# gvtulder/elasticdeform

Hardware: AMD Instinct MI355X
Metric: Mvoxels/s fwd+grad, 256^3 fp32 order=3 (higher is better)
Workload: dtype f32; 1 GPU; cfg2: 3D 256x256x256 float32, 5x5x5 grid sigma 5, order 3, mode mirror, prefilter on, deform_grid + deform_grid_gradient per step, one volume per GPU; parallelism=1 volume per GPU, no collective

## Files before the change

### elasticdeform_amd/csrc/deform_k1z.hip

```cpp
#include <hip/hip_runtime.h>

#include <cstring>
#include <type_traits>

#include "ed_device.h"
#include "ed_gridfilter.h"
#include "ed_params.h"
#include "ed_tile.h"
#include "ed_workspace.h"
#include "ed_zwalk.h"

namespace ed {
namespace tile {

#ifdef EDHIP_K1_STATS
__device__ unsigned long long g_k1z_stats[8];
#define ZSTAT(K, N) atomicAdd(&g_k1z_stats[K], (unsigned long long)(N))
#else
#define ZSTAT(K, N) do { } while (0)
#endif

namespace {


enum : int {
    kZAny = 1,
    kZStaged = 2,
    kZFast = 4,
    kZDma = 8,
    kZXin = 16,
    kZZYin = 32,
    kZUnfit = 64,
    kZGen = 128,
};
struct ZRecU {
    int b0z, b0y, b0x, flags, pitch, ez, ey, ex, goff, plane;
};
typedef int zv8i __attribute__((ext_vector_type(8)));
typedef const __attribute__((address_space(4))) zv8i* crec_p;
__device__ __forceinline__ ZRecU zrec_unpack(const zv8i& v)
{
    ZRecU r;
    r.b0z = v[0];
    r.b0y = v[1];
    r.b0x = v[2];
    r.flags = v[3];
    r.pitch = (v[3] >> 8) & 255;
    r.ez = v[4] & 1023;
    r.ey = (v[4] >> 10) & 1023;
    r.ex = (int)((unsigned)v[4] >> 20);
    r.goff = v[5];
    r.plane = r.ey * r.pitch;
    return r;
}
__device__ __forceinline__ ZRecU zrec_load(crec_p p)
{
    const zv8i v = *p;
    return zrec_unpack(v);
}

__host__ __device__ __forceinline__ int zctl(int parity, int list, int xcd) { return (parity * 2 + list) * 8 + xcd; }

#define ED_RED6(CTRL)                                      \
    "v_min_i32_dpp %0, %0, %0 " CTRL "\n\t"                \
    "v_min_i32_dpp %1, %1, %1 " CTRL "\n\t"                \
    "v_min_i32_dpp %2, %2, %2 " CTRL "\n\t"                \
    "v_max_i32_dpp %3, %3, %3 " CTRL "\n\t"                \
    "v_max_i32_dpp %4, %4, %4 " CTRL "\n\t"                \
    "v_max_i32_dpp %5, %5, %5 " CTRL "\n\t"
__device__ __forceinline__ void zrow_box(int (&lo)[3], int (&hi)[3])
{
    asm volatile("s_nop 1\n\t"
                 ED_RED6("quad_perm:[1,0,3,2] row_mask:0xf bank_mask:0xf")
                 ED_RED6("quad_perm:[2,3,0,1] row_mask:0xf bank_mask:0xf")
                 ED_RED6("row_half_mirror row_mask:0xf bank_mask:0xf")
                 ED_RED6("row_mirror row_mask:0xf bank_mask:0xf")
                 : "+v"(lo[0]), "+v"(lo[1]), "+v"(lo[2]), "+v"(hi[0]), "+v"(hi[1]), "+v"(hi[2]));
}
#undef ED_RED6
__device__ __forceinline__ int zuni(int v) { return __builtin_amdgcn_readfirstlane(v); }
__device__ __forceinline__ void zlds_barrier() { asm volatile("s_waitcnt lgkmcnt(0)\n\ts_barrier" ::: "memory"); }
__device__ __forceinline__ void zdma_barrier() { asm volatile("s_waitcnt vmcnt(0) lgkmcnt(0)\n\ts_barrier" ::: "memory"); }
__device__ __forceinline__ void zglds16(const float* g, float* lds)
{
    __builtin_amdgcn_global_load_lds((const __attribute__((address_space(1))) void*)g,
                                     (__attribute__((address_space(3))) void*)lds, 16, 0, 0);
}
template <bool OUT16>
__device__ __forceinline__ void zstore_out(float* img, long long off, float val, int io16)
{
    if constexpr (OUT16)
        reinterpret_cast<unsigned short*>(img)[off] = (unsigned short)narrow16(val, io16);
    else
        __builtin_nontemporal_store(val, img + off);
}

__device__ __forceinline__ void zaxis_entry(const GridGeom& g, int a, int oi, double* w, int* idx)
{
    const double cp = control_coordinate(g.ncp[a], (int64_t)oi + g.off[a], g.in_len[a]);
    const int64_t start = window_start(cp, 3);
    const bool edge = start < 0 || start + 3 >= g.ncp[a];
    spline_weights(cp, 3, w);
#pragma unroll
    for (int l = 0; l < 4; ++l)
        idx[l] = edge ? mirror_i32((int)start + l, (int)g.ncp[a]) : (int)start + l;
}

constexpr int kGeoBlock = 256;
constexpr int kGeoWaves = kGeoBlock / 64;
__global__ __launch_bounds__(kGeoBlock) void k1z_geo_kernel(const GridGeom g, const HotGeom hg, const ZGeom zg,
                                                          const GridPrefilter gp)
{
    extern __shared__ __attribute__((aligned(16))) char smem[];
    const int tid = threadIdx.x;
// ... 190 lines not shown
            lo[h] = (int)floor(cr - slack[h]);
            hi[h] = (int)floor(cr + slack[h]);
        }
        bool out_of_fast = false;
#pragma unroll
        for (int h = 0; h < 3; ++h)
            out_of_fast = out_of_fast || lo[h] < ((order & 1) ? 0 : 1) || hi[h] > hg.in_len[h] - 2;
        const bool fast = nz == kT && ny == kT && nx == kT && !__any(out_of_fast);
        zrow_box(lo, hi);
        int* dst = sBox + (tz * 8 + (lane >> 4)) * 8;
        if ((lane & 15) == 0) {
#pragma unroll
            for (int h = 0; h < 3; ++h) {
                dst[h] = lo[h];
                dst[4 + h] = hi[h];
            }
        }
        if (lane == 0)
            dst[3] = fast ? 1 : 0;
        if (!fast) {
            bool cst = false;
#pragma unroll
            for (int h = 0; h < 3; ++h) {
                double m = c[h];
                if (!(m >= 0.0 && m <= (double)(hg.in_len[h] - 1)))
                    m = map_coordinate_fast(m, hg.in_len[h], hg.mode, hg.period[h], hg.inv_period[h]);
                cst = cst || !(m > -1.0);
                const double mr = (order & 1) ? m : m + 0.5;
                lo[h] = (int)floor(mr - slack[h]);
                hi[h] = (int)floor(mr + slack[h]);
            }
            if (cst) {
#pragma unroll
                for (int h = 0; h < 3; ++h) {
                    lo[h] = 0x7fffffff;
                    hi[h] = (int)0x80000000;
                }
            }
            zrow_box(lo, hi);
            if ((lane & 15) == 0) {
#pragma unroll
                for (int h = 0; h < 3; ++h) {
                    dst[32 + h] = lo[h];
                    dst[36 + h] = hi[h];
                }
            }
        }
    }
    __syncthreads();
    ZTICK(6);
    for (int tz = tid; tz < hg.tiles[0] && !ED_DBG(hg.dbg, 1 << 27); tz += kGeoBlock) {
        const int tile_id = sample * hg.ntiles + (tz * hg.tiles[1] + ty) * hg.tiles[2] + tx;
        int cls = 0;
        bool hint0 = false, half_fit[2] = {false, false};
#pragma unroll 1
        for (int part = 0; part < 3; ++part) {
            const int* sb = sBox + tz * 64;
            const bool fast = sb[3] != 0;
            const int r0 = part == 2 ? 2 : 0, r1 = part == 1 ? 2 : 3;
            int blo[3], bhi[3];
            bool any = true;
#pragma unroll
            for (int h = 0; h < 3; ++h) {
                int rlo = 0x7fffffff, rhi = (int)0x80000000, lo = 0x7fffffff, hi = (int)0x80000000;
                for (int r = r0; r <= r1; ++r) {
                    rlo = min(rlo, sb[r * 8 + h]);
                    rhi = max(rhi, sb[r * 8 + 4 + h]);
                    lo = min(lo, sb[(fast ? 0 : 32) + r * 8 + h]);
                    hi = max(hi, sb[(fast ? 0 : 32) + r * 8 + 4 + h]);
                }
                if (!fast) {
                    any = any && hi >= lo;
                    const int lowfold = hg.mode == EDHIP_MODE_REFLECT ? -1 : 0;
                    if (rlo < ((order & 1) ? 0 : 1) && rhi >= lowfold)
                        lo = min(lo, lowfold);
                    if (rhi > hg.in_len[h] - 2 && rlo <= hg.in_len[h] - 1)
                        hi = max(hi, hg.in_len[h] - 1);
                }
                blo[h] = lo - H;
                bhi[h] = hi - H + order + (h == 2 ? kPadX : 0);
            }
            if (!any) {
                blo[0] = blo[1] = blo[2] = 0;
                bhi[0] = bhi[1] = bhi[2] = -1;
            }
            any = bhi[0] >= blo[0] && bhi[1] >= blo[1] && bhi[2] >= blo[2];
            unsigned ext[3];
#pragma unroll
            for (int h = 0; h < 3; ++h)
                ext[h] = (unsigned)bhi[h] - (unsigned)blo[h] + 1u;
            const int pitch = ext[2] <= 16u ? 16 : (ext[2] <= 24u ? 24 : (ext[2] <= 32u ? 32 : (ext[2] <= 48u ? 48 : 0)));
            const bool sane = any && ext[0] < 1024u && ext[1] < 1024u;
            const int nrows = sane ? (int)(ext[0] * ext[1]) : 0;
            const bool fits = sane && pitch > 0 && nrows * pitch <= hg.box_cap;
            const bool dma = fits && blo[2] >= 0 && blo[2] + pitch + 1 <= hg.in_len[2];
            const bool xin = fits && blo[2] >= 0 && blo[2] + (int)ext[2] <= hg.in_len[2];
            const bool zyin = fits && blo[0] >= 0 && blo[0] + (int)ext[0] <= hg.in_len[0] && blo[1] >= 0 &&
                              blo[1] + (int)ext[1] <= hg.in_len[1];
            const bool fastA = part == 0 && fast && fits && dma && zyin;
            const int flags = (any ? kZAny : 0) | (fits ? kZStaged : 0) | (fastA ? kZFast : kZGen) | (dma ? kZDma : 0) |
                              (xin ? kZXin : 0) | (zyin ? kZZYin : 0) | (any && !fits ? kZUnfit : 0);
            const int4 w0 = make_int4(blo[0], blo[1], blo[2], flags | (pitch << 8));
            const int4 w1 = make_int4(sane ? (int)(ext[0] | (ext[1] << 10) | (ext[2] << 20)) : 0,
                                      (dma && zyin) ? blo[0] * hg.vol_sz + blo[1] * hg.vol_sy + blo[2] : 0, 0, 0);
            if (part == 0) {
                hint0 = any && !(sane && pitch > 0 && nrows * pitch <= hg.small_cap);
                cls = (flags & kZUnfit) ? 3 : ((flags & kZFast) ? 1 : 2);
                int4* dst = reinterpret_cast<int4*>(zg.recs + (size_t)tile_id * 8);
                dst[0] = w0;
                dst[1] = w1;
                if (hg.boxes) {
                    int* bx = hg.boxes + (size_t)tile_id * 8;
#pragma unroll
                    for (int h = 0; h < 3; ++h) {
                        bx[h] = blo[h];
                        bx[3 + h] = bhi[h] - ((h == 2 && any) ? kPadX : 0);
                    }
                }
                if (cls != 3)
                    break;
            } else {
                half_fit[part - 1] = fits || !any;
                int4* dst = reinterpret_cast<int4*>(zg.recs_half + ((size_t)tile_id * 2 + (part - 1)) * 8);
                dst[0] = w0;
                dst[1] = w1;
            }
        }
        const bool split = cls == 3 && half_fit[0] && half_fit[1];
        ZSTAT(cls == 3 ? (split ? 6 : 5) : (cls == 1 ? 3 : 4), 1);
        sCls[tz] = cls | (split ? 4 : 0) | (hint0 ? 8 : 0);
    }
    __syncthreads();
    ZTICK(7);
    {
        const int zstrips = (hg.tiles[0] + zg.strip_tiles - 1) / zg.strip_tiles;
        if (tid < 4)
            sCnt[tid] = 0;
        __syncthreads();
        int slotG = -1, slotF = -1, sidv = 0;
        if (tid < zstrips) {
            int info = 0;
            bool g = false, f = false;
            for (int k = 0; k < zg.strip_tiles && tid * zg.strip_tiles + k < hg.tiles[0]; ++k) {
                const int c = sCls[tid * zg.strip_tiles + k];
                info |= c << (4 * k);
                g = g || (c & 3) == 2 || (c & 7) == 7;
                f = f || (c & 7) == 3;
            }
            const size_t sid = (size_t)sample * zg.nstrips + ((size_t)tid * hg.tiles[1] + ty) * hg.tiles[2] + tx;
            sidv = (int)sid;
            zg.sinfo[sid] = info;
            zg.missed[sid] = f ? 2 : 0;
            if (g)
                slotG = atomicAdd(&sCnt[0], 1);
            if (f)
                slotF = atomicAdd(&sCnt[1], 1);
        }
        __syncthreads();
        const int xcd = (tx + ty + sample) & 7;
        if (tid == 0) {
            sCnt[2] = sCnt[0] ? atomicAdd(&zg.ctl[zctl(zg.parity, 0, xcd)], sCnt[0]) : 0;
            sCnt[3] = sCnt[1] ? atomicAdd(&zg.ctl[zctl(zg.parity, 1, xcd)], sCnt[1]) : 0;
        }
        if (blockIdx.x == 0 && sample == 0 && tid < 16)
            zg.ctl[zctl(1 - zg.parity, tid >> 3, tid & 7)] = 0;
        __syncthreads();
        if (slotG >= 0)
            zg.list_g[(size_t)(sCnt[2] + slotG) * 8 + xcd] = sidv;
        if (slotF >= 0)
            zg.list_f[(size_t)(sCnt[3] + slotF) * 8 + xcd] = sidv;
    }
    ZTICK(8);
#undef ZTICK
}


struct ZVox {
    int addr[2];
    float frac[2][3];
    int flg;
};
struct ZStrip {
    int tz0, ty, tx, ntile, sample, id;
};
__device__ __forceinline__ bool k1z_strip(int total_strips, int nstrips, int tiles_z, int tiles_y, int tiles_x, int strip_tiles, int deal,
                                          ZStrip& sp, int b)
{
    const int x = b & 7, j = b >> 3;
    const int r = j / deal;
    int s = (r * 8 + ((x + r) & 7)) * deal + (j - r * deal);
    if (s >= total_strips)
        return false;
    sp.id = s;
    sp.sample = s / nstrips;
    s -= sp.sample * nstrips;
    sp.tx = s % tiles_x;
    s /= tiles_x;
    sp.ty = s % tiles_y;
    sp.tz0 = (s / tiles_y) * strip_tiles;
    sp.ntile = min(strip_tiles, tiles_z - sp.tz0);
    return true;
}
inline unsigned k1z_grid(int total_strips, int deal)
{
    const int chunks = (total_strips + deal - 1) / deal;
    return (unsigned)(((chunks + 7) / 8) * 8 * deal);
}

template <int ORDER, int PITCH>
__device__ __forceinline__ float k1z_gather(const float* bp, int plane, int pitch_rt, const float* w0, const float* w1, const float* w2)
{
    constexpr int NT = ORDER + 1;
    constexpr int NTX = NT + (NT & 1);
    float a0 = 0.f;
#pragma unroll
    for (int l0 = 0; l0 < NT; ++l0) {
        const float* pp = bp + l0 * plane;
        float a1 = 0.f;
#pragma unroll
        for (int l1 = 0; l1 < NT; ++l1) {
            const float* rp = pp + l1 * (PITCH ? PITCH : pitch_rt);
// ... 1 lines not shown
#pragma unroll
            for (int l2 = 0; l2 < NTX; l2 += 2) {
                const float2 pr = *reinterpret_cast<const float2*>(rp + l2);
                ED_NO_DS_MERGE();
                a2 = fmaf(w2[l2], pr.x, a2);
                a2 = fmaf(w2[l2 + 1], pr.y, a2);
            }
            a1 = fmaf(w1[l1], a2, a1);
        }
        a0 = fmaf(w0[l0], a1, a0);
    }
    return a0;
}
template <int ORDER>
__device__ __forceinline__ float k1z_voxel(const char* smem, int addr, const float (&frac)[3], int pitch, int plane)
{
    constexpr int NT = ORDER + 1;
    constexpr int NTX = NT + (NT & 1);
    float f0 = frac[0], f1 = frac[1], f2 = frac[2];
    asm volatile("" : "+v"(f0), "+v"(f1), "+v"(f2));
    float w0[NT], w1[NT], w2[NTX];
    weights_from_frac<float, ORDER>(f0, w0);
    weights_from_frac<float, ORDER>(f1, w1);
    weights_from_frac<float, ORDER>(f2, w2);
    if (NT & 1)
        w2[NT] = 0.f;
    const float* bp = reinterpret_cast<const float*>(smem + addr);
    return pitch == 16 ? k1z_gather<ORDER, 16>(bp, plane, 16, w0, w1, w2) : k1z_gather<ORDER, 0>(bp, plane, pitch, w0, w1, w2);
}

struct ZFast {
    const float* vol;
    float* img;
    const double* r;
    const AxTab* zt;
    const int* recs;
    const int* recs_half;
    int* missed;
    int* hint;
    const int* sinfo;
    const int* list_g;
    int* list_f;
    int* ctl;
    int parity;
    const long long* steps;
    long long vol_bstride, img_bstride, r_bstride;
    int vol_sy, vol_sz, img_sy, img_sz;
    int box_cap, tiles_y, tiles_x, tiles_z, strip_tiles, nstrips, total_strips, ntiles;
    int rcol_bytes, out_y, out_x;
    int kz0, ky0, kx0;
    int io16, nsteps, deal;
    int dbg;
    double aff[12];
};

template <int ORDER, bool AFFINE, bool OUT16, bool STEPS>
__device__ __forceinline__ void k1z_fast_body(const ZFast& a, const int vblock)
{
    constexpr int NT = ORDER + 1;
    constexpr int kPadX = NT & 1;
    constexpr int NTX = NT + kPadX;
    extern __shared__ __attribute__((aligned(16))) char smem[];
    ZStrip sp;
    if (!k1z_strip(a.total_strips, a.nstrips, a.tiles_z, a.tiles_y, a.tiles_x, a.strip_tiles, a.deal, sp, vblock))
        return;
    const int tid = threadIdx.x;
    const int lane = tid & 63;
    const int wave = zuni(tid >> 6);
    const int io16 = OUT16 ? a.io16 : 0;
    const int ntile = sp.ntile;
    const size_t tile_step = (size_t)a.tiles_y * a.tiles_x;
    crec_p rec0 = (crec_p)(const void*)a.recs + ((size_t)sp.sample * a.ntiles + ((size_t)sp.tz0 * a.tiles_y + sp.ty) * a.tiles_x + sp.tx);
    const int sinfo = ((cint_p)(const void*)a.sinfo)[sp.id];
    if (a.hint && tid == 0) {
        const int nh = __builtin_popcount((unsigned)sinfo & 0x88888888u);
        if (nh)
            atomicAdd(a.hint, nh);
    }
    auto next_fast = [&](int t) {
        for (++t; t < ntile; ++t)
            if (((sinfo >> (4 * t)) & 3) == 1)
                break;
        return t;
    };
    int ti = next_fast(-1);
    if (ti >= ntile)
        return;

    const int box_cap = a.box_cap;
    const int odd_shift = (box_cap - 1) * 4;
    float* box0 = reinterpret_cast<float*>(smem);
    float* box1 = box0 + box_cap;
    const int vol_sz = a.vol_sz, vol_sy = a.vol_sy, img_sz = a.img_sz;

    const int yy = lane >> 3, xx = lane & 7;
    const int oy = sp.ty * kT + yy, ox = sp.tx * kT + xx;
    const int obase = oy * a.img_sy + ox;
    const float* __restrict__ vol = a.vol + sp.sample * a.vol_bstride;
    float* img = a.img + sp.sample * a.img_bstride;
    const char* rcol = reinterpret_cast<const char*>(a.r + sp.sample * a.r_bstride) +
                       ((size_t)min(oy, a.out_y - 1) * a.out_x + min(ox, a.out_x - 1)) * (size_t)a.rcol_bytes;
    const int ky = AFFINE ? a.ky0 : oy + a.ky0;
    const int kx = AFFINE ? a.kx0 : ox + a.kx0;
    const int kz0 = a.kz0;
    double Pyx[3];
#pragma unroll
    for (int h = 0; h < 3; ++h)
// ... 59 lines not shown
            const int rx = ci[2] + dx;
            bad |= (rz | ry | rx) | ((ez - rz) | (ey - ry) | (ex - rx));
            const int off = __mul24(rz, rc.plane) + (__mul24(ry, rc.pitch) + rx);
            vs.addr[i] = __mul24(off & 1, odd_shift) + off * 4;
        }
    };

    cll_p steps = (cll_p)(const void*)a.steps;
    ZVox cur, nxt;
    ZRecU rc = zrec_load(rec0 + (size_t)ti * tile_step), rn = rc;
    {
        const ZEnt ze[2] = {k1z_entry(zt, (sp.tz0 + ti) * kT + wave), k1z_entry(zt, (sp.tz0 + ti) * kT + wave + 4)};
        tile_coords(ti, rc, ze, cur);
    }
    while (ti < ntile) {
        const int tn = next_fast(ti);
        const int tl = tn < ntile ? tn : ti;
        const zv8i rnv = *(rec0 + (size_t)tl * tile_step);
        const ZEnt zn[2] = {k1z_entry(zt, (sp.tz0 + tl) * kT + wave), k1z_entry(zt, (sp.tz0 + tl) * kT + wave + 4)};
        if (!ED_DBG(a.dbg, 1 << 18))
            stage(rc, vol + (STEPS ? steps[0] : 0));
        if (tn < ntile) {
            rn = zrec_unpack(rnv);
            tile_coords(tn, rn, zn, nxt);
        }
        const long long ozoff = (long long)((sp.tz0 + ti) * kT + wave) * img_sz + obase;
        const int nsteps = STEPS ? a.nsteps : 1;
        for (int ss = 0; ss < nsteps; ++ss) {
            if (STEPS && ss > 0)
                stage(rc, vol + steps[2 * ss]);
            zdma_barrier();
#pragma unroll
            for (int i = 0; i < 2; ++i) {
                const float val = ED_DBG(a.dbg, 1 << 17) ? cur.frac[i][0] + cur.frac[i][1] + cur.frac[i][2] + __int_as_float(cur.addr[i])
                                                         : k1z_voxel<ORDER>(smem, cur.addr[i], cur.frac[i], rc.pitch, rc.plane);
                if (!ED_DBG(a.dbg, 1 << 20) || val == 123.456f)
                    zstore_out<OUT16>(img, (STEPS ? steps[2 * ss + 1] : 0) + ozoff + (long long)(4 * i) * img_sz, val, io16);
            }
            zlds_barrier();
        }
        cur = nxt;
        rc = rn;
        ti = tn;
    }
    if (__any(bad < 0) && lane == 0) {
        if (atomicOr(a.missed + sp.id, 1) == 0) {
            const int xcd = vblock & 7;
            a.list_f[(size_t)atomicAdd(a.ctl + zctl(a.parity, 1, xcd), 1) * 8 + xcd] = sp.id;
        }
    }
}

template <int ORDER, bool AFFINE, bool OUT16, bool STEPS>
__device__ __forceinline__ void k1z_gen_body(const ZFast& a, czgen_p zn, const int vblock, const int ngen)
{
    constexpr int NT = ORDER + 1;
    constexpr int kPadX = NT & 1;
    constexpr int NTX = NT + kPadX;
    extern __shared__ __attribute__((aligned(16))) char smem[];
    const int tid = threadIdx.x;
    const int lane = tid & 63;
    const int wave = zuni(tid >> 6);
    const int io16 = OUT16 ? a.io16 : 0;
    const int xcd = vblock & 7, nper = ngen >> 3;
    const int nwork = ((cint_p)(const void*)a.ctl)[zctl(a.parity, 0, xcd)];
    if ((vblock >> 3) >= nwork)
        return;
    const int box_cap = a.box_cap;
    const int odd_shift = (box_cap - 1) * 4;
    float* box0 = reinterpret_cast<float*>(smem);
    float* box1 = box0 + box_cap;
    const int vol_sz = a.vol_sz, vol_sy = a.vol_sy, img_sz = a.img_sz;
    const size_t tile_step = (size_t)a.tiles_y * a.tiles_x;
    cdbl_p zt = (cdbl_p)(const void*)a.zt;
    cll_p steps = (cll_p)(const void*)a.steps;
    const int nsteps = STEPS ? a.nsteps : 1;
    const int yy = lane >> 3, xx = lane & 7;

    for (int work = vblock >> 3; work < nwork; work += nper) {
        ZStrip sp;
        {
            int sid = ((cint_p)(const void*)a.list_g)[(size_t)work * 8 + xcd];
            sp.id = sid;
            sp.sample = sid / a.nstrips;
            sid -= sp.sample * a.nstrips;
            sp.tx = sid % a.tiles_x;
            sid /= a.tiles_x;
            sp.ty = sid % a.tiles_y;
            sp.tz0 = (sid / a.tiles_y) * a.strip_tiles;
            sp.ntile = min(a.strip_tiles, a.tiles_z - sp.tz0);
        }
        const int ntile = sp.ntile;
        crec_p rec0 = (crec_p)(const void*)a.recs + ((size_t)sp.sample * a.ntiles + ((size_t)sp.tz0 * a.tiles_y + sp.ty) * a.tiles_x + sp.tx);
        const int sinfo = ((cint_p)(const void*)a.sinfo)[sp.id];
        crec_p rech0 = (crec_p)(const void*)a.recs_half + ((size_t)sp.sample * a.ntiles + ((size_t)sp.tz0 * a.tiles_y + sp.ty) * a.tiles_x + sp.tx) * 2;
        if (tid == 0)
            ZSTAT(7, 1);
        if (work != (vblock >> 3))
            zlds_barrier();
        const int oy = sp.ty * kT + yy, ox = sp.tx * kT + xx;
        const int obase = oy * a.img_sy + ox;
        const float* __restrict__ vol = a.vol + sp.sample * a.vol_bstride;
        float* img = a.img + sp.sample * a.img_bstride;
        const char* rcol = reinterpret_cast<const char*>(a.r + sp.sample * a.r_bstride) +
                           ((size_t)min(oy, a.out_y - 1) * a.out_x + min(ox, a.out_x - 1)) * (size_t)a.rcol_bytes;
        double Pyx[3];
#pragma unroll
        for (int h = 0; h < 3; ++h)
            Pyx[h] = AFFINE ? fma(zn->aff[h * 4 + 2], (double)ox, fma(zn->aff[h * 4 + 1], (double)oy, zn->aff[h * 4 + 3] + zn->offd[h])) : 0.0;
        ZTaps tp;
        tp.key[0] = tp.key[1] = tp.key[2] = tp.key[3] = -1;
        auto stage = [&](const ZRecU& rc, const float* src) {
            const int flags = rc.flags;
            if (!(flags & kZStaged))
                return;
            const int by = rc.ey, pitch = rc.pitch;
            if (flags & kZDma) {
                const int cpr = pitch >> 2, RW = 64 / cpr;
                const int lr = (lane * (65536 / cpr + 1)) >> 16, q = lane - lr * cpr;
                const float* g0 = src + (rc.b0x + 4 * q);
                for (int zrow = wave; zrow < rc.ez; zrow += 4) {
                    const float* gp = g0 + (long long)mirror_i32(rc.b0z + zrow, zn->in_len[0]) * vol_sz;
                    const int lrow0 = zrow * by;
                    for (int y0 = 0; y0 < by; y0 += RW) {
                        if (lr < RW && y0 + lr < by) {
                            const float* g = gp + (long long)mirror_i32(rc.b0y + y0 + lr, zn->in_len[1]) * vol_sy;
                            zglds16(g, box0 + (lrow0 + y0) * pitch);
                            zglds16(g + 1, box1 + (lrow0 + y0) * pitch);
                        }
                    }
                }
            } else {
                const int nrows = rc.ez * rc.ey;
                const float inv_by = __frcp_rn((float)by);
                const int sub = tid & 7;
                for (int rb = tid >> 3; rb < nrows; rb += 2 * (kBlock / 8)) {
                    for (int x0 = sub; x0 < rc.ex; x0 += 16) {
                        float val[2][2];
#pragma unroll
                        for (int u = 0; u < 2; ++u) {
                            const int r = min(rb + u * (kBlock / 8), nrows - 1);
                            const int zrow = (int)(((float)r + 0.5f) * inv_by), yr = r - zrow * by;
                            const int zs = mirror_i32(rc.b0z + zrow, zn->in_len[0]);
                            const int ys = mirror_i32(rc.b0y + yr, zn->in_len[1]);
                            const float* rowp = src + (zs * vol_sz + ys * vol_sy);
#pragma unroll
                            for (int j = 0; j < 2; ++j) {
                                const int xi = min(x0 + 8 * j, rc.ex - 1);
                                const int xs = mirror_i32(rc.b0x + xi, zn->in_len[2]);
                                val[u][j] = rowp[xs];
                            }
                        }
#pragma unroll
                        for (int u = 0; u < 2; ++u) {
                            const int r = rb + u * (kBlock / 8);
#pragma unroll
                            for (int j = 0; j < 2; ++j) {
                                const int xi = x0 + 8 * j;
                                if (r < nrows && xi < rc.ex) {
                                    box0[r * pitch + xi] = val[u][j];
                                    if (xi > 0)
                                        box1[r * pitch + xi - 1] = val[u][j];
                                }
                            }
                        }
                    }
                }
            }
        };
        int bad = 0;
        auto tile_coords = [&](int t, int mask, const ZRecU& rc, ZVox& vs) {
            const int ez = rc.ez - NT, ey = rc.ey - NT, ex = rc.ex - NTX;
            const bool staged = (rc.flags & kZStaged) != 0;
            vs.flg = 0;
#pragma unroll
            for (int i = 0; i < 2; ++i) {
                if (!(mask & (1 << i)))
                    continue;
                const int oz = (sp.tz0 + t) * kT + wave + 4 * i;
                double zw[4];
                k1z_slice(zt, rcol, min(oz, zn->out_len[0] - 1), tp, zw);
                double d[3];
                k1z_disp(tp, zw, d);
                const int b[3] = {oz + zn->off[0], oy + zn->off[1], ox + zn->off[2]};
                double P[3] = {0.0, 0.0, 0.0};
                if (AFFINE) {
#pragma unroll
                    for (int h = 0; h < 3; ++h)
                        P[h] = fma(zn->aff[h * 4 + 0], (double)oz, Pyx[h]);
                }
                int start[3];
                const bool cst = k1z_coords<ORDER, AFFINE>(zn, d, b, P, start, vs.frac[i]);
                const bool valid = oz < zn->out_len[0] && oy < zn->out_len[1] && ox < zn->out_len[2];
                const int rz = start[0] - rc.b0z, ry = start[1] - rc.b0y, rx = start[2] - rc.b0x;
                if (valid && !cst)
                    bad |= staged ? (rz | ry | rx) | ((ez - rz) | (ey - ry) | (ex - rx)) : -1;
                vs.flg |= (valid && !cst && staged ? 1 << i : 0) | (valid && (cst || staged) ? 4 << i : 0);
                const int off = __mul24(rz, rc.plane) + (__mul24(ry, rc.pitch) + rx);
                vs.addr[i] = __mul24(off & 1, odd_shift) + off * 4;
            }
        };
        {
            auto next_item = [&](int it) {
                int t = it >> 1;
                if (it >= 0 && (it & 1) == 0 && ((sinfo >> (4 * t)) & 7) == 7)
                    return it + 1;
                for (++t; t < ntile; ++t) {
                    const int c = (sinfo >> (4 * t)) & 7;
                    if ((c & 3) == 2 || c == 7)
                        break;
                }
                return 2 * t;
            };
            auto item_rec = [&](int it) {
                const int t = it >> 1;
                const bool split = ((sinfo >> (4 * t)) & 7) == 7;
                return zrec_load(split ? rech0 + ((size_t)t * tile_step * 2 + (it & 1)) : rec0 + (size_t)t * tile_step);
            };
            auto item_mask = [&](int it) { return ((sinfo >> (4 * (it >> 1))) & 7) == 7 ? 1 << (it & 1) : 3; };
            ZVox cur, nxt;
            int it = next_item(-2);
            ZRecU rc = item_rec(it < 2 * ntile ? it : 0), rn = rc;
            if (it < 2 * ntile)
                tile_coords(it >> 1, item_mask(it), rc, cur);
            while (it < 2 * ntile) {
                stage(rc, vol + (STEPS ? steps[0] : 0));
                const int in = next_item(it);
                if (in < 2 * ntile) {
                    rn = item_rec(in);
                    tile_coords(in >> 1, item_mask(in), rn, nxt);
                }
                const bool staged = (rc.flags & kZStaged) != 0;
                const long long ozoff = (long long)((sp.tz0 + (it >> 1)) * kT + wave) * img_sz + obase;
                for (int ss = 0; ss < nsteps; ++ss) {
                    if (STEPS && ss > 0)
                        stage(rc, vol + steps[2 * ss]);
                    if (staged)
                        zdma_barrier();
#pragma unroll
                    for (int i = 0; i < 2; ++i) {
                        if (!(cur.flg & (4 << i)))
                            continue;
                        float val = zn->cval;
                        if (cur.flg & (1 << i))
                            val = k1z_voxel<ORDER>(smem, cur.addr[i], cur.frac[i], rc.pitch, rc.plane);
                        zstore_out<OUT16>(img, (STEPS ? steps[2 * ss + 1] : 0) + ozoff + (long long)(4 * i) * img_sz, val, io16);
                    }
                    if (staged)
                        zlds_barrier();
                }
                cur = nxt;
                rc = rn;
                it = in;
            }
        }
        if (__any(bad < 0) && lane == 0) {
            if (atomicOr(a.missed + sp.id, 1) == 0) {
                const int xcd = vblock & 7;
                a.list_f[(size_t)atomicAdd(a.ctl + zctl(a.parity, 1, xcd), 1) * 8 + xcd] = sp.id;
            }
        }
    }
}

template <int ORDER, bool AFFINE, bool OUT16, bool STEPS>
__global__ __launch_bounds__(kBlock, 4) void k1z_tile_kernel(const ZFast a, czgen_p zn, const int ngen, const int every)
{
    const int row = (int)(blockIdx.x >> 3), xcd = (int)(blockIdx.x & 7);
    const int gen_rows = ngen >> 3;
    const int gens_before = min((row + 1) / every, gen_rows);
    const bool is_gen = gens_before > 0 && (row + 1) % every == 0 && (row + 1) / every <= gen_rows;
    if (is_gen)
        k1z_gen_body<ORDER, AFFINE, OUT16, STEPS>(a, zn, (gens_before - 1) * 8 + xcd, ngen);
    else
        k1z_fast_body<ORDER, AFFINE, OUT16, STEPS>(a, (row - gens_before) * 8 + xcd);
}

template <int ORDER, bool AFFINE, bool OUT16, bool STEPS>
__global__ __launch_bounds__(kBlock) void k1z_fix_kernel(const ZFast a, czgen_p zn)
{
    constexpr int NT = ORDER + 1;
    constexpr int kPadX = NT & 1;
    const int tid = threadIdx.x;
    const int lane = tid & 63;
    const int wave = zuni(tid >> 6);
    const int io16 = OUT16 ? a.io16 : 0;
    const int xcd = (int)(blockIdx.x & 7), nper = (int)(gridDim.x >> 3);
    const int nwork = ((cint_p)(const void*)a.ctl)[zctl(a.parity, 1, xcd)];
    if ((int)(blockIdx.x >> 3) >= nwork)
        return;
    const int vol_sz = a.vol_sz, vol_sy = a.vol_sy, img_sz = a.img_sz;
    const size_t tile_step = (size_t)a.tiles_y * a.tiles_x;
    cdbl_p zt = (cdbl_p)(const void*)a.zt;
    cll_p steps = (cll_p)(const void*)a.steps;
    const int nsteps = STEPS ? a.nsteps : 1;
    const int yy = lane >> 3, xx = lane & 7;

    for (int work = blockIdx.x >> 3; work < nwork; work += nper) {
        ZStrip sp;
        {
            int sid = ((cint_p)(const void*)a.list_f)[(size_t)work * 8 + xcd];
            sp.id = sid;
            sp.sample = sid / a.nstrips;
            sid -= sp.sample * a.nstrips;
            sp.tx = sid % a.tiles_x;
            sid /= a.tiles_x;
            sp.ty = sid % a.tiles_y;
            sp.tz0 = (sid / a.tiles_y) * a.strip_tiles;
            sp.ntile = min(a.strip_tiles, a.tiles_z - sp.tz0);
        }
        const int ntile = sp.ntile;
        crec_p rec0 = (crec_p)(const void*)a.recs + ((size_t)sp.sample * a.ntiles + ((size_t)sp.tz0 * a.tiles_y + sp.ty) * a.tiles_x + sp.tx);
        crec_p rech0 = (crec_p)(const void*)a.recs_half + ((size_t)sp.sample * a.ntiles + ((size_t)sp.tz0 * a.tiles_y + sp.ty) * a.tiles_x + sp.tx) * 2;
        const int sinfo = ((cint_p)(const void*)a.sinfo)[sp.id];
        const bool missed = (((cint_p)(const void*)a.missed)[sp.id] & 1) != 0;
        if (!STEPS && false)
            (void)steps;
        const int oy = sp.ty * kT + yy, ox = sp.tx * kT + xx;
        const int obase = oy * a.img_sy + ox;
        const float* __restrict__ vol = a.vol + sp.sample * a.vol_bstride;
        float* img = a.img + sp.sample * a.img_bstride;
        const char* rcol = reinterpret_cast<const char*>(a.r + sp.sample * a.r_bstride) +
                           ((size_t)min(oy, a.out_y - 1) * a.out_x + min(ox, a.out_x - 1)) * (size_t)a.rcol_bytes;
        double Pyx[3];
#pragma unroll
        for (int h = 0; h < 3; ++h)
            Pyx[h] = AFFINE ? fma(zn->aff[h * 4 + 2], (double)ox, fma(zn->aff[h * 4 + 1], (double)oy, zn->aff[h * 4 + 3] + zn->offd[h])) : 0.0;
        ZTaps tp;
// ... 38 lines not shown
                                  rx = (gen ? st[2] : raw[2]) - rc.b0x;
                        const bool inside = rz >= 0 && rz + NT <= rc.ez && ry >= 0 && ry + NT <= rc.ey && rx >= 0 &&
                                            rx + NT + kPadX <= rc.ex;
                        if (inside)
                            continue;
                    }
                    int tap[3][NT];
                    float w[3][NT];
#pragma unroll
                    for (int h = 0; h < 3; ++h) {
                        weights_from_frac<float, ORDER>(fr[h], w[h]);
                        const int stride = h == 0 ? vol_sz : (h == 1 ? vol_sy : 1);
#pragma unroll
                        for (int l = 0; l < NT; ++l)
                            tap[h][l] = mirror_i32(st[h] + l, zn->in_len[h]) * stride;
                    }
                    const long long ooff = (long long)oz * img_sz + obase;
                    ZSTAT(whole ? 2 : 1, 1);
                    for (int ss = 0; ss < nsteps; ++ss) {
                        float val = zn->cval;
                        if (!cst) {
                            const float* src = vol + (STEPS ? steps[2 * ss] : 0);
                            float a0 = 0.f;
#pragma unroll
                            for (int l0 = 0; l0 < NT; ++l0) {
                                float a1 = 0.f;
#pragma unroll
                                for (int l1 = 0; l1 < NT; ++l1) {
                                    const float* p1 = src + (tap[0][l0] + tap[1][l1]);
                                    float a2 = 0.f;
#pragma unroll
                                    for (int l2 = 0; l2 < NT; ++l2)
                                        a2 = fmaf(w[2][l2], p1[tap[2][l2]], a2);
                                    a1 = fmaf(w[1][l1], a2, a1);
                                }
                                a0 = fmaf(w[0][l0], a1, a0);
                            }
                            val = a0;
                        }
                        zstore_out<OUT16>(img, (STEPS ? steps[2 * ss + 1] : 0) + ooff, val, io16);
                    }
                }
            }
        }
    }
}

template <int ORDER, bool AFFINE, bool OUT16, bool STEPS>
hipError_t launch_k1z_kernels(const ZFast& zf, const void* znp, unsigned ngen, unsigned nfix, size_t lds, hipStream_t stream)
{
    const unsigned nfast = k1z_grid(zf.total_strips, zf.deal);
    const unsigned fast_rows = nfast >> 3, gen_rows = ngen >> 3;
    unsigned every = gen_rows ? fast_rows / gen_rows + 1 : 2;
    if (every < 2)
        every = 2;
    hipLaunchKernelGGL((k1z_tile_kernel<ORDER, AFFINE, OUT16, STEPS>), dim3(nfast + ngen), dim3(kBlock), lds, stream, zf, (czgen_p)znp,
                       (int)ngen, (int)every);
    hipError_t e = hipGetLastError();
    if (e != hipSuccess)
        return e;
    hipLaunchKernelGGL((k1z_fix_kernel<ORDER, AFFINE, OUT16, STEPS>), dim3(nfix, 2 * zf.strip_tiles), dim3(kBlock), 0, stream, zf, (czgen_p)znp);
    return hipGetLastError();
}
template <int ORDER, bool AFFINE, bool OUT16>
hipError_t launch_k1z_variant(const ZFast& zf, const void* zn, unsigned ngen, unsigned nfix, size_t lds, hipStream_t stream,
                              bool steps)
{
    return steps ? launch_k1z_kernels<ORDER, AFFINE, OUT16, true>(zf, zn, ngen, nfix, lds, stream)
                 : launch_k1z_kernels<ORDER, AFFINE, OUT16, false>(zf, zn, ngen, nfix, lds, stream);
}
template <int ORDER>
hipError_t launch_k1z_order(const HotGeom& hg, const ZFast& zf, const void* zn, unsigned ngen, unsigned nfix, size_t lds, hipStream_t stream)
{
    const bool steps = hg.nstep != 0;
    if (hg.io16)
        return hg.has_affine ? launch_k1z_variant<ORDER, true, true>(zf, zn, ngen, nfix, lds, stream, steps)
                             : launch_k1z_variant<ORDER, false, true>(zf, zn, ngen, nfix, lds, stream, steps);
    return hg.has_affine ? launch_k1z_variant<ORDER, true, false>(zf, zn, ngen, nfix, lds, stream, steps)
                         : launch_k1z_variant<ORDER, false, false>(zf, zn, ngen, nfix, lds, stream, steps);
}

}

size_t k1z_lds_bytes(int* box_cap, bool large)
{
    size_t budget = large ? 52 * 1024 : 31 * 1024;
    if (const char* kb = ed_env("EDHIP_ZKB"))
        budget = (size_t)atoi(kb) * 1024;
    size_t cap = budget / 8;
    cap = ((cap - 56) / 64) * 64 + 56;
    *box_cap = (int)cap;
    return 2 * 4 * cap;
}

size_t k1z_geo_lds_bytes(const GridGeom& g, const HotGeom& hg)
{
    const size_t ngrid = 3 * (size_t)g.ncp[0] * (size_t)g.ncp[1] * (size_t)g.ncp[2];
    return 8 * ngrid + 8 * 64 * 3 * (size_t)g.ncp[0] + 16 * sizeof(AxTab) + 3 * kGeoWaves * 8 + (sizeof(AxTab) * 4 + 4 + 256) * (size_t)hg.tiles[0] + 16;
}

size_t k1z_r_bytes(const GridGeom& g) { return 8 * (size_t)g.out_len[1] * (size_t)g.out_len[2] * 4 * (size_t)g.ncp[0]; }

bool k1z_supported(const GridGeom& g)
{
    const size_t ngrid = 3 * (size_t)g.ncp[0] * (size_t)g.ncp[1] * (size_t)g.ncp[2];
    const size_t tiles_z = (size_t)((g.out_len[0] + kT - 1) / kT);
    return ngrid <= 4096 && g.ncp[0] <= 16 &&
           8 * ngrid + 8 * 64 * 3 * (size_t)g.ncp[0] + 16 * sizeof(AxTab) + 3 * kGeoWaves * 8 + (sizeof(AxTab) * 4 + 4 + 256) * tiles_z + 16 <= 60 * 1024;
}

hipError_t launch_k1z_geo(const GridGeom& g, const HotGeom& hg, const ZGeom& zg, const GridPrefilter& gp, int nbatch,
                          hipStream_t stream)
{
    hipLaunchKernelGGL(k1z_geo_kernel, dim3((unsigned)(hg.tiles[1] * hg.tiles[2]), (unsigned)nbatch), dim3(kGeoBlock),
                       k1z_geo_lds_bytes(g, hg), stream, g, hg, zg, gp);
    if (ed_env("EDHIP_GEO_TWICE"))
        hipLaunchKernelGGL(k1z_geo_kernel, dim3((unsigned)(hg.tiles[1] * hg.tiles[2]), (unsigned)nbatch), dim3(kGeoBlock),
                           k1z_geo_lds_bytes(g, hg), stream, g, hg, zg, gp);
    return hipGetLastError();
}

hipError_t launch_k1z(const HotGeom& hg, const ZGeom& zg, int order, size_t lds, hipStream_t stream)
{
    ZFast zf;
    memset(&zf, 0, sizeof(zf));
    zf.vol = hg.vol_r;
    zf.img = hg.img_w;
    zf.r = zg.r;
    zf.zt = zg.zt;
    zf.recs = zg.recs;
    zf.recs_half = zg.recs_half;
    zf.missed = zg.missed;
    zf.hint = hg.hint;
    zf.sinfo = zg.sinfo;
    zf.list_g = zg.list_g;
    zf.list_f = zg.list_f;
    zf.ctl = zg.ctl;
    zf.parity = zg.parity;
    zf.steps = zg.steps;
    zf.vol_bstride = hg.vol_bstride;
    zf.img_bstride = hg.img_bstride;
    zf.r_bstride = zg.r_bstride;
    zf.vol_sy = hg.vol_sy;
    zf.vol_sz = hg.vol_sz;
    zf.img_sy = hg.img_sy;
    zf.img_sz = hg.img_sz;
    zf.box_cap = hg.box_cap;
    zf.tiles_z = hg.tiles[0];
    zf.tiles_y = hg.tiles[1];
    zf.tiles_x = hg.tiles[2];
    zf.strip_tiles = zg.strip_tiles;
    zf.nstrips = zg.nstrips;
    zf.total_strips = zg.total_strips;
    zf.ntiles = hg.ntiles;
    zf.rcol_bytes = 32 * zg.ncpz;
    zf.out_y = hg.out_len[1];
    zf.out_x = hg.out_len[2];
    const int H = order / 2;
    zf.kz0 = (hg.has_affine ? 0 : hg.off[0]) - H;
    zf.ky0 = (hg.has_affine ? 0 : hg.off[1]) - H;
    zf.kx0 = (hg.has_affine ? 0 : hg.off[2]) - H;
    zf.io16 = hg.io16;
    zf.nsteps = (int)hg.nsteps;
    zf.dbg = hg.dbg;
    zf.deal = 4 * hg.tiles[2];
    while (zf.deal > 1 && zg.total_strips < 16 * zf.deal)
        zf.deal >>= 1;
    if (const char* dl = ed_env("EDHIP_ZDEAL"))
        zf.deal = atoi(dl) >= 1 ? atoi(dl) : zf.deal;
    for (int h = 0; h < 3; ++h) {
        for (int k = 0; k < 3; ++k)
            zf.aff[h * 4 + k] = hg.affine[h * 4 + k];
        zf.aff[h * 4 + 3] = hg.affine[h * 4 + 3] + (double)hg.off[h];
    }
    const void* zn = zg.zgen;
    unsigned ngen = (unsigned)(zg.total_strips < 1280 ? ((zg.total_strips + 7) / 8) * 8 : 1280);
    if (const char* ng = ed_env("EDHIP_ZNGEN"))
        ngen = (unsigned)((atoi(ng) + 7) / 8 * 8);
    const unsigned nfix = (unsigned)(zg.total_strips < 512 ? ((zg.total_strips + 7) / 8) * 8 : 512);
    switch (order) {
    case 1: return launch_k1z_order<1>(hg, zf, zn, ngen, nfix, lds, stream);
    case 2: return launch_k1z_order<2>(hg, zf, zn, ngen, nfix, lds, stream);
    case 3: return launch_k1z_order<3>(hg, zf, zn, ngen, nfix, lds, stream);
    default: return hipErrorNotSupported;
    }
}

#ifdef EDHIP_K1_STATS
extern "C" int edhip_debug_k1z_stats(unsigned long long* out8)
{
    unsigned long long z[8] = {0, 0, 0, 0, 0, 0, 0, 0};
    if (hipMemcpyFromSymbol(out8, HIP_SYMBOL(g_k1z_stats), sizeof(z)) != hipSuccess)
        return 1;
    return hipMemcpyToSymbol(HIP_SYMBOL(g_k1z_stats), z, sizeof(z)) != hipSuccess;
}
#endif

}
}
```

Measured before the change: 25930 Mvoxels/s.

## Split gen strips into heavy/light lists with atomic work-stealing cursor and row-form staging

Classifies general-path strips as heavy (slow non-DMA staged tiles, splits, or many gen tiles) or light, and packs heavy ones from the front of the gen list and light ones from the back. Gen blocks now pull work dynamically through a per-XCD atomic cursor with a double-buffered LDS prefetch of the next index, replacing the static strided assignment. A new row-form staging path for non-DMA tiles uses 16-byte global-to-LDS loads plus an in-LDS fixup for mirrored edge columns. These changes aim to reduce load imbalance and slow per-element staging. In exchange they add atomics, extra barriers and more complex control flow, and a debug-timing path guarded by an experiments macro.

```diff
diff --git a/elasticdeform_amd/csrc/deform_k1z.hip b/elasticdeform_amd/csrc/deform_k1z.hip
--- a/elasticdeform_amd/csrc/deform_k1z.hip
+++ b/elasticdeform_amd/csrc/deform_k1z.hip
@@ -59,7 +59,8 @@
     return zrec_unpack(v);
 }
 
-__host__ __device__ __forceinline__ int zctl(int parity, int list, int xcd) { return (parity * 2 + list) * 8 + xcd; }
+enum : int { kZHeavy = 0, kZFix = 1, kZLight = 2, kZCursor = 3 };
+__host__ __device__ __forceinline__ int zctl(int parity, int word, int xcd) { return (parity * 4 + word) * 8 + xcd; }
 
 #define ED_RED6(CTRL)                                      \
     "v_min_i32_dpp %0, %0, %0 " CTRL "\n\t"                \
@@ -356,7 +357,7 @@
     for (int tz = tid; tz < hg.tiles[0] && !ED_DBG(hg.dbg, 1 << 27); tz += kGeoBlock) {
         const int tile_id = sample * hg.ntiles + (tz * hg.tiles[1] + ty) * hg.tiles[2] + tx;
         int cls = 0;
-        bool hint0 = false, half_fit[2] = {false, false};
+        bool hint0 = false, slow0 = false, half_fit[2] = {false, false};
 #pragma unroll 1
         for (int part = 0; part < 3; ++part) {
             const int* sb = sBox + tz * 64;
@@ -409,6 +410,7 @@
                                       (dma && zyin) ? blo[0] * hg.vol_sz + blo[1] * hg.vol_sy + blo[2] : 0, 0, 0);
             if (part == 0) {
                 hint0 = any && !(sane && pitch > 0 && nrows * pitch <= hg.small_cap);
+                slow0 = fits && !dma;
                 cls = (flags & kZUnfit) ? 3 : ((flags & kZFast) ? 1 : 2);
                 int4* dst = reinterpret_cast<int4*>(zg.recs + (size_t)tile_id * 8);
                 dst[0] = w0;
@@ -432,45 +434,54 @@
         }
         const bool split = cls == 3 && half_fit[0] && half_fit[1];
         ZSTAT(cls == 3 ? (split ? 6 : 5) : (cls == 1 ? 3 : 4), 1);
-        sCls[tz] = cls | (split ? 4 : 0) | (hint0 ? 8 : 0);
+        sCls[tz] = cls | (split ? 4 : 0) | (hint0 ? 8 : 0) | ((cls == 2 && slow0) || split ? 16 : 0);
     }
     __syncthreads();
     ZTICK(7);
     {
         const int zstrips = (hg.tiles[0] + zg.strip_tiles - 1) / zg.strip_tiles;
+        int* sCntL = reinterpret_cast<int*>(sMax);
         if (tid < 4)
             sCnt[tid] = 0;
+        if (tid < 2)
+            sCntL[tid] = 0;
         __syncthreads();
-        int slotG = -1, slotF = -1, sidv = 0;
+        int slotG = -1, slotL = -1, slotF = -1, sidv = 0;
         if (tid < zstrips) {
-            int info = 0;
-            bool g = false, f = false;
+            int info = 0, ngen = 0;
+            bool slow = false, f = false;
             for (int k = 0; k < zg.strip_tiles && tid * zg.strip_tiles + k < hg.tiles[0]; ++k) {
                 const int c = sCls[tid * zg.strip_tiles + k];
-                info |= c << (4 * k);
-                g = g || (c & 3) == 2 || (c & 7) == 7;
+                info |= (c & 15) << (4 * k);
+                ngen += ((c & 3) == 2 || (c & 7) == 7) ? 1 : 0;
+                slow = slow || (c & 16) != 0;
                 f = f || (c & 7) == 3;
             }
             const size_t sid = (size_t)sample * zg.nstrips + ((size_t)tid * hg.tiles[1] + ty) * hg.tiles[2] + tx;
             sidv = (int)sid;
             zg.sinfo[sid] = info;
             zg.missed[sid] = f ? 2 : 0;
-            if (g)
+            if (ngen && (slow || ngen >= 3) && !ED_DBG(hg.dbg, 1 << 13))
                 slotG = atomicAdd(&sCnt[0], 1);
+            else if (ngen)
+                slotL = atomicAdd(&sCntL[0], 1);
             if (f)
                 slotF = atomicAdd(&sCnt[1], 1);
         }
         __syncthreads();
         const int xcd = (tx + ty + sample) & 7;
         if (tid == 0) {
-            sCnt[2] = sCnt[0] ? atomicAdd(&zg.ctl[zctl(zg.parity, 0, xcd)], sCnt[0]) : 0;
-            sCnt[3] = sCnt[1] ? atomicAdd(&zg.ctl[zctl(zg.parity, 1, xcd)], sCnt[1]) : 0;
-        }
-        if (blockIdx.x == 0 && sample == 0 && tid < 16)
+            sCnt[2] = sCnt[0] ? atomicAdd(&zg.ctl[zctl(zg.parity, kZHeavy, xcd)], sCnt[0]) : 0;
+            sCnt[3] = sCnt[1] ? atomicAdd(&zg.ctl[zctl(zg.parity, kZFix, xcd)], sCnt[1]) : 0;
+            sCntL[1] = sCntL[0] ? atomicAdd(&zg.ctl[zctl(zg.parity, kZLight, xcd)], sCntL[0]) : 0;
+        }
+        if (blockIdx.x == 0 && sample == 0 && tid < 32)
             zg.ctl[zctl(1 - zg.parity, tid >> 3, tid & 7)] = 0;
         __syncthreads();
         if (slotG >= 0)
             zg.list_g[(size_t)(sCnt[2] + slotG) * 8 + xcd] = sidv;
+        if (slotL >= 0)
+            zg.list_g[(size_t)(zg.total_strips - 1 - (sCntL[1] + slotL)) * 8 + xcd] = sidv;
         if (slotF >= 0)
             zg.list_f[(size_t)(sCnt[3] + slotF) * 8 + xcd] = sidv;
     }
@@ -578,7 +589,13 @@
     int io16, nsteps, deal;
     int dbg;
     double aff[12];
+#ifdef EDHIP_EXPERIMENTS
+    unsigned long long* dbgbuf;
+#endif
 };
+#ifdef EDHIP_EXPERIMENTS
+constexpr size_t kZDbgBase = (size_t)1 << 16;
+#endif
 
 template <int ORDER, bool AFFINE, bool OUT16, bool STEPS>
 __device__ __forceinline__ void k1z_fast_body(const ZFast& a, const int vblock)
@@ -744,7 +761,7 @@
 }
 
 template <int ORDER, bool AFFINE, bool OUT16, bool STEPS>
-__device__ __forceinline__ void k1z_gen_body(const ZFast& a, czgen_p zn, const int vblock, const int ngen)
+__device__ __forceinline__ void k1z_gen_body(const ZFast& a, czgen_p zn, const int vblock)
 {
     constexpr int NT = ORDER + 1;
     constexpr int kPadX = NT & 1;
@@ -754,11 +771,19 @@
     const int lane = tid & 63;
     const int wave = zuni(tid >> 6);
     const int io16 = OUT16 ? a.io16 : 0;
-    const int xcd = vblock & 7, nper = ngen >> 3;
-    const int nwork = ((cint_p)(const void*)a.ctl)[zctl(a.parity, 0, xcd)];
-    if ((vblock >> 3) >= nwork)
+    const int xcd = vblock & 7;
+    const int nheavy = ((cint_p)(const void*)a.ctl)[zctl(a.parity, kZHeavy, xcd)];
+    const int nwork = nheavy + ((cint_p)(const void*)a.ctl)[zctl(a.parity, kZLight, xcd)];
+    if (ED_DBG(a.dbg, 1 << 15) || nwork == 0)
         return;
     const int box_cap = a.box_cap;
+    int* cursor = a.ctl + zctl(a.parity, kZCursor, xcd);
+    volatile int* sNext = reinterpret_cast<volatile int*>(smem + 8 * (size_t)box_cap);
+    int fetched = 0, turn = 0;
+    if (tid == 0)
+        sNext[0] = atomicAdd(cursor, 1);
+    zlds_barrier();
+    int work = zuni(sNext[0]);
     const int odd_shift = (box_cap - 1) * 4;
     float* box0 = reinterpret_cast<float*>(smem);
     float* box1 = box0 + box_cap;
@@ -769,10 +794,13 @@
     const int nsteps = STEPS ? a.nsteps : 1;
     const int yy = lane >> 3, xx = lane & 7;
 
-    for (int work = vblock >> 3; work < nwork; work += nper) {
+    while (work < nwork) {
+        if (tid == 0)
+            fetched = atomicAdd(cursor, 1);
         ZStrip sp;
         {
-            int sid = ((cint_p)(const void*)a.list_g)[(size_t)work * 8 + xcd];
+            const int slot = work < nheavy ? work : a.total_strips - 1 - (work - nheavy);
+            int sid = ((cint_p)(const void*)a.list_g)[(size_t)slot * 8 + xcd];
             sp.id = sid;
             sp.sample = sid / a.nstrips;
             sid -= sp.sample * a.nstrips;
@@ -788,8 +816,10 @@
         crec_p rech0 = (crec_p)(const void*)a.recs_half + ((size_t)sp.sample * a.ntiles + ((size_t)sp.tz0 * a.tiles_y + sp.ty) * a.tiles_x + sp.tx) * 2;
         if (tid == 0)
             ZSTAT(7, 1);
-        if (work != (vblock >> 3))
-            zlds_barrier();
+#ifdef EDHIP_EXPERIMENTS
+        const unsigned long long dbg_t0 = a.dbgbuf ? wall_clock64() : 0;
+        int dbg_kind = 0;
+#endif
         const int oy = sp.ty * kT + yy, ox = sp.tx * kT + xx;
         const int obase = oy * a.img_sy + ox;
         const float* __restrict__ vol = a.vol + sp.sample * a.vol_bstride;
@@ -802,6 +832,38 @@
             Pyx[h] = AFFINE ? fma(zn->aff[h * 4 + 2], (double)ox, fma(zn->aff[h * 4 + 1], (double)oy, zn->aff[h * 4 + 3] + zn->offd[h])) : 0.0;
         ZTaps tp;
         tp.key[0] = tp.key[1] = tp.key[2] = tp.key[3] = -1;
+        auto row_form = [&](const ZRecU& rc) {
+            const int W = zn->in_len[2];
+            const int m = mirror_i32(rc.b0x + min(lane, rc.ex - 1), W);
+            const int mlo = wave_min(m), mhi = wave_max(m);
+            return W >= 4 && mlo >= min(max(rc.b0x, 0), W - 4) && mhi < min(max(rc.b0x + rc.pitch, 4), W);
+        };
+        bool rowf = false;
+        auto stage_fix = [&](const ZRecU& rc) {
+            const int W = zn->in_len[2], pitch = rc.pitch, by = rc.ey;
+            const int cpr = pitch >> 2, lpr = 2 * cpr, RW = 64 / lpr;
+            const int lr = (lane * (65536 / lpr + 1)) >> 16, rem = lane - lr * lpr;
+            const int c = rem >= cpr ? 1 : 0, q = rem - c * cpr;
+            const int s = rc.b0x + 4 * q + c;
+            const bool moved = (s < 0 || s + 4 > W) && lr < RW;
+            int loc[4];
+#pragma unroll
+            for (int j = 0; j < 4; ++j) {
+                const int m = mirror_i32(rc.b0x + min(4 * q + c + j, rc.ex - 1), W);
+                const int qs = min(max((m - rc.b0x) >> 2, 0), cpr - 1);
+                loc[j] = 4 * qs + min(max(m - min(max(rc.b0x + 4 * qs, 0), W - 4), 0), 3);
+            }
+            asm volatile("s_waitcnt vmcnt(0)" ::: "memory");
+            for (int zrow = wave; zrow < rc.ez; zrow += 4) {
+                for (int y0 = 0; y0 < by; y0 += RW) {
+                    if (moved && y0 + lr < by) {
+                        float* row = box0 + (zrow * by + y0 + lr) * pitch;
+                        const float4 v = make_float4(row[loc[0]], row[loc[1]], row[loc[2]], row[loc[3]]);
+                        *reinterpret_cast<float4*>(row + c * box_cap + 4 * q) = v;
+                    }
+                }
+            }
+        };
         auto stage = [&](const ZRecU& rc, const float* src) {
             const int flags = rc.flags;
             if (!(flags & kZStaged))
@@ -822,6 +884,22 @@
                         }
                     }
                 }
+            } else if ((rowf = row_form(rc))) {
+                const int W = zn->in_len[2];
+                const int cpr = pitch >> 2, RW = 64 / cpr;
+                const int lr = (lane * (65536 / cpr + 1)) >> 16, q = lane - lr * cpr;
+                const int s0 = min(max(rc.b0x + 4 * q, 0), W - 4), s1 = min(max(rc.b0x + 4 * q + 1, 0), W - 4);
+                for (int zrow = wave; zrow < rc.ez; zrow += 4) {
+                    const float* gp = src + (long long)mirror_i32(rc.b0z + zrow, zn->in_len[0]) * vol_sz;
+                    const int lrow0 = zrow * by;
+                    for (int y0 = 0; y0 < by; y0 += RW) {
+                        if (lr < RW && y0 + lr < by) {
+                            const float* g = gp + (long long)mirror_i32(rc.b0y + y0 + lr, zn->in_len[1]) * vol_sy;
+                            zglds16(g + s0, box0 + (lrow0 + y0) * pitch);
+                            zglds16(g + s1, box1 + (lrow0 + y0) * pitch);
+                        }
+                    }
+                }
             } else {
                 const int nrows = rc.ez * rc.ey;
                 const float inv_by = __frcp_rn((float)by);
@@ -916,6 +994,9 @@
             if (it < 2 * ntile)
                 tile_coords(it >> 1, item_mask(it), rc, cur);
             while (it < 2 * ntile) {
+#ifdef EDHIP_EXPERIMENTS
+                dbg_kind = (dbg_kind + 1) | ((rc.flags & (kZStaged | kZDma)) == kZStaged ? 256 : 0);
+#endif
                 stage(rc, vol + (STEPS ? steps[0] : 0));
                 const int in = next_item(it);
                 if (in < 2 * ntile) {
@@ -927,6 +1008,8 @@
                 for (int ss = 0; ss < nsteps; ++ss) {
                     if (STEPS && ss > 0)
                         stage(rc, vol + steps[2 * ss]);
+                    if (staged && !(rc.flags & kZDma) && rowf)
+                        stage_fix(rc);
                     if (staged)
                         zdma_barrier();
 #pragma unroll
@@ -948,10 +1031,25 @@
         }
         if (__any(bad < 0) && lane == 0) {
             if (atomicOr(a.missed + sp.id, 1) == 0) {
-                const int xcd = vblock & 7;
-                a.list_f[(size_t)atomicAdd(a.ctl + zctl(a.parity, 1, xcd), 1) * 8 + xcd] = sp.id;
-            }
-        }
+                a.list_f[(size_t)atomicAdd(a.ctl + zctl(a.parity, kZFix, xcd), 1) * 8 + xcd] = sp.id;
+            }
+        }
+#ifdef EDHIP_EXPERIMENTS
+        if (a.dbgbuf && tid == 0) {
+            const unsigned long long nrec = atomicAdd(a.dbgbuf + kZDbgBase, 1ull);
+            unsigned long long* rec = a.dbgbuf + kZDbgBase + 8 + 4 * (nrec < 40000 ? nrec : 40000);
+            rec[0] = (unsigned long long)(unsigned)sp.id | ((unsigned long long)(dbg_kind & 255) << 32) |
+                     ((unsigned long long)(dbg_kind >> 8) << 40) | ((unsigned long long)xcd << 48);
+            rec[1] = dbg_t0;
+            rec[2] = wall_clock64();
+            rec[3] = (unsigned long long)work;
+        }
+#endif
+        turn ^= 1;
+        if (tid == 0)
+            sNext[turn] = fetched;
+        zlds_barrier();
+        work = zuni(sNext[turn]);
     }
 }
 
@@ -962,10 +1060,22 @@
     const int gen_rows = ngen >> 3;
     const int gens_before = min((row + 1) / every, gen_rows);
     const bool is_gen = gens_before > 0 && (row + 1) % every == 0 && (row + 1) / every <= gen_rows;
+#ifdef EDHIP_EXPERIMENTS
+    if (a.dbgbuf && blockIdx.x == 0 && threadIdx.x == 0)
+        a.dbgbuf[kZDbgBase + 3] = wall_clock64();
+#endif
     if (is_gen)
-        k1z_gen_body<ORDER, AFFINE, OUT16, STEPS>(a, zn, (gens_before - 1) * 8 + xcd, ngen);
-    else
+        k1z_gen_body<ORDER, AFFINE, OUT16, STEPS>(a, zn, (gens_before - 1) * 8 + xcd);
+    else if (!ED_DBG(a.dbg, 1 << 14))
         k1z_fast_body<ORDER, AFFINE, OUT16, STEPS>(a, (row - gens_before) * 8 + xcd);
+#ifdef EDHIP_EXPERIMENTS
+    if (a.dbgbuf && threadIdx.x == 0) {
+        const unsigned long long now = wall_clock64();
+        if (!is_gen)
+            atomicMax(a.dbgbuf + kZDbgBase + 1, now);
+        atomicMax(a.dbgbuf + kZDbgBase + 2, now);
+    }
+#endif
 }
 
 template <int ORDER, bool AFFINE, bool OUT16, bool STEPS>
@@ -1110,6 +1220,8 @@
     const unsigned nfast = k1z_grid(zf.total_strips, zf.deal);
     const unsigned fast_rows = nfast >> 3, gen_rows = ngen >> 3;
     unsigned every = gen_rows ? fast_rows / gen_rows + 1 : 2;
+    if (const char* ev = ed_env("EDHIP_ZEVERY"))
+        every = (unsigned)atoi(ev);
     if (every < 2)
         every = 2;
     hipLaunchKernelGGL((k1z_tile_kernel<ORDER, AFFINE, OUT16, STEPS>), dim3(nfast + ngen), dim3(kBlock), lds, stream, zf, (czgen_p)znp,
@@ -1148,7 +1260,7 @@
     size_t cap = budget / 8;
     cap = ((cap - 56) / 64) * 64 + 56;
     *box_cap = (int)cap;
-    return 2 * 4 * cap;
+    return 2 * 4 * cap + 16;
 }
 
 size_t k1z_geo_lds_bytes(const GridGeom& g, const HotGeom& hg)
@@ -1221,6 +1333,9 @@
     zf.io16 = hg.io16;
     zf.nsteps = (int)hg.nsteps;
     zf.dbg = hg.dbg;
+#ifdef EDHIP_EXPERIMENTS
+    zf.dbgbuf = hg.dbgbuf;
+#endif
     zf.deal = 4 * hg.tiles[2];
     while (zf.deal > 1 && zg.total_strips < 16 * zf.deal)
         zf.deal >>= 1;
```

Result: faster. 26380 Mvoxels/s, median of 6 (+1.7%).
